# LayerXcom/zero-chain

Measured on NVIDIA H100. Metric: g1_msm_mops_2^20, higher is better.
Workload: dtype u32-limb Montgomery (Fq 12x32, Fr 8x32), integer

## Files before the change

zero_chain_b200/csrc/engine.cu:

```cuda
#define ZK_SEMI_HOT 1
#include "internal.h"
#include "msm_driver.cuh"

using namespace zkmsm;

static thread_local char g_err[512] = "";
void zk_set_error(const char *fmt, ...) {
    va_list ap; va_start(ap, fmt); vsnprintf(g_err, sizeof(g_err), fmt, ap); va_end(ap);
    (void)cudaGetLastError();
}
extern "C" const char *zk_last_error(void) { return g_err; }
extern "C" const char *zk_version(void) { return "zkb200 0.1 (sm_90a)"; }
extern "C" int zk_device_count(void) {
    int n = 0;
    if (cudaGetDeviceCount(&n) != cudaSuccess) { cudaGetLastError(); return 0; }
    return n;
}
int zk_use_device(zk_ctx *ctx) { ZK_CUDA(cudaSetDevice(ctx->device)); return ZK_OK; }

extern "C" int zk_ctx_create(int device, void *stream, zk_ctx **out) {
    if (!out) { zk_set_error("zk_ctx_create: out is NULL"); return ZK_ERR_INVALID; }
    int n = zk_device_count();
    if (n == 0) { zk_set_error("no CUDA device: libzkb200 has no CPU fallback"); return ZK_ERR_CUDA; }
    if (device < 0 || device >= n) { zk_set_error("device %d out of range (%d devices)", device, n); return ZK_ERR_INVALID; }
    ZK_CUDA(cudaSetDevice(device));
    zk_ctx *c = new zk_ctx();
    c->device = device;
    if (stream) { c->stream = (cudaStream_t)stream; c->own_stream = false; }
    else { ZK_CUDA(cudaStreamCreateWithFlags(&c->stream, cudaStreamNonBlocking)); c->own_stream = true; }
    cudaDeviceProp prop;
    ZK_CUDA(cudaGetDeviceProperties(&prop, device));
    c->sm_count = prop.multiProcessorCount;
    ZK_CUDA(cudaMalloc(&c->d_err, 32 * sizeof(int)));
    ZK_CUDA(cudaMemsetAsync(c->d_err, 0, 32 * sizeof(int), c->stream));
    c->h_pinned_cap = 1 << 20;
    ZK_CUDA(cudaMallocHost(&c->h_pinned, c->h_pinned_cap));
    *out = c;
    return ZK_OK;
}
extern "C" void zk_ctx_destroy(zk_ctx *c) {
    if (!c) return;
    if (c->aux) { zk_ctx_destroy(c->aux); c->aux = nullptr; }
    if (c->aux2) { zk_ctx_destroy(c->aux2); c->aux2 = nullptr; }
    if (c->aux3) { zk_ctx_destroy(c->aux3); c->aux3 = nullptr; }
    cudaSetDevice(c->device);
    cudaStreamSynchronize(c->stream);
    DevBuf *bufs[] = {&c->scalars, &c->digits, &c->tile_hist, &c->tile_off, &c->sizes, &c->bucket_off, &c->task_off, &c->scan_scratch,
                      &c->sorted, &c->partials, &c->buckets, &c->red_part, &c->red_x, &c->result, &c->out_bytes, &c->stage_a, &c->stage_b,
                      &c->stage_c, &c->ntt_tmp, &c->g_a, &c->g_b, &c->g_c, &c->g_h, &c->g_scal, &c->g_misc,
                      &c->aff_pts0, &c->aff_pts1, &c->aff_scratch, &c->aff_off0, &c->aff_off1, &c->aff_sizes0, &c->aff_sizes1, &c->aff_srcs, &c->aff_tot, &c->red_rows, &c->g_scal2, &c->g_scal3, &c->sorted2, &c->coarse_off, &c->coarse_sizes, &c->task_order, &c->len_hist, &c->heavy_list, &c->red_tmp,
                      &c->v_pts, &c->v_stat, &c->v_coef, &c->v_f, &c->v_part, &c->v_io, &c->v_jj,
                      &c->eg_table, &c->eg_index, &c->jm, &c->bal, &c->bal_io};
    for (DevBuf *b : bufs) b->release();
    for (NttSlot &sl : c->ntt_slots) { sl.w.release(); sl.g.release(); sl.gi.release(); sl.consts.release(); }
    if (c->tail) { cudaStreamSynchronize(c->tail); cudaStreamDestroy(c->tail); cudaEventDestroy(c->ev_front); cudaEventDestroy(c->ev_tail); }
    if (c->d_err) cudaFree(c->d_err);
    if (c->h_pinned) cudaFreeHost(c->h_pinned);
    if (c->own_stream) cudaStreamDestroy(c->stream);
    delete c;
}
extern "C" int zk_ctx_set_opt(zk_ctx *c, int opt, long value) {
    if (!c) { zk_set_error("zk_ctx_set_opt: NULL ctx"); return ZK_ERR_INVALID; }
    for (zk_ctx *x : {c, c->aux, c->aux2, c->aux3}) {
        if (!x) continue;
        if (opt == ZK_OPT_AFFINE_MIN_ENTRIES) x->opts.ba_min_entries = value;
        else if (opt == ZK_OPT_AFFINE_LEVELS) x->opts.ba_levels = value;
        else if (opt == ZK_OPT_VERIFY_LANES) x->opts.verify_lanes = value;
        else { zk_set_error("zk_ctx_set_opt: unknown option %d", opt); return ZK_ERR_INVALID; }
    }
    return ZK_OK;
}
extern "C" int zk_ctx_sync(zk_ctx *c) { ZK_TRY(zk_use_device(c)); return zk_check_err_flag(c); }
extern "C" void *zk_ctx_stream(zk_ctx *c) { return (void *)c->stream; }

int zk_check_err_flag(zk_ctx *ctx) {
    int e[3] = {0, 0, 0};
    ZK_CUDA(cudaMemcpyAsync(e, ctx->d_err, sizeof(e), cudaMemcpyDeviceToHost, ctx->stream));
    ZK_CUDA(cudaStreamSynchronize(ctx->stream));
    if (e[0] || e[1] || e[ZK_ERR_SLOT_ACCOUNT]) {
        ZK_CUDA(cudaMemsetAsync(ctx->d_err, 0, sizeof(e), ctx->stream));
        if (e[0]) { zk_set_error("scalar not canonical (>= r)"); return ZK_ERR_NOT_CANONICAL; }
        if (e[ZK_ERR_SLOT_ACCOUNT]) {
            zk_set_error("account %u: a stored ciphertext fails Ciphertext::read", ~(uint32_t)e[ZK_ERR_SLOT_ACCOUNT]);
// ... 333 lines not shown
```

zero_chain_b200/csrc/internal.h:

```cpp
#pragma once
#include <cuda_runtime.h>
#include <stdarg.h>
#include <stdint.h>
#include <stdio.h>
#include <string.h>
#include <string>
#include <vector>
#include "../../include/zkb200.h"

void zk_set_error(const char *fmt, ...);
#define ZK_CUDA(call)                                                                                  \
    do {                                                                                               \
        cudaError_t e__ = (call);                                                                      \
        if (e__ != cudaSuccess) {                                                                      \
            zk_set_error("%s:%d: %s -> %s", __FILE__, __LINE__, #call, cudaGetErrorString(e__));       \
            return ZK_ERR_CUDA;                                                                        \
        }                                                                                              \
    } while (0)
#define ZK_TRY(call) do { int r__ = (call); if (r__ != ZK_OK) return r__; } while (0)

struct DevBuf {
    void *p = nullptr;
    size_t cap = 0;
    int reserve(size_t bytes) {
// ... 5 lines not shown
        if (e != cudaSuccess) { zk_set_error("cudaMalloc(%zu) failed: %s", want, cudaGetErrorString(e)); return ZK_ERR_CUDA; }
        cap = want;
        return ZK_OK;
    }
    void release() { if (p) cudaFree(p); p = nullptr; cap = 0; }
    template <class T> T *as() const { return reinterpret_cast<T *>(p); }
};

struct Carve {
    uint8_t *base = nullptr;
    size_t off = 0;
    template <class T> T *take(size_t count) {
        T *p = reinterpret_cast<T *>(base ? base + off : nullptr);
        off += (count * sizeof(T) + 255) & ~(size_t)255;
        return p;
    }
};

struct NttSlot { unsigned log_n = 0; bool valid = false; uint64_t last_use = 0; DevBuf w, g, gi, consts; };

struct zk_opts {
    long ba_min_entries = 1l << 22;
    long ba_levels = -1;
    long verify_lanes = 1;
};

struct zk_ctx {
    zk_opts opts;
    int device = 0;
    cudaStream_t stream = nullptr;
    bool own_stream = false;
    int sm_count = 0;
    int *d_err = nullptr;
    DevBuf aff_pts0, aff_pts1, aff_scratch, aff_off0, aff_off1, aff_sizes0, aff_sizes1, aff_srcs, aff_tot;
    DevBuf scalars, digits, tile_hist, tile_off, sizes, bucket_off, task_off, scan_scratch, sorted, partials, buckets, red_part, red_x, red_rows, sorted2, coarse_off, coarse_sizes, task_order, len_hist, heavy_list, red_tmp, result, out_bytes;
    bool len_hist_zeroed = false;
    DevBuf stage_a, stage_b, stage_c;
    DevBuf ntt_tmp;
    NttSlot ntt_slots[4];
    uint64_t ntt_clock = 0;
    bool ntt_attr_done = false;
    DevBuf g_a, g_b, g_c, g_h, g_scal, g_misc;
    DevBuf v_pts, v_stat, v_coef, v_f, v_part, v_io;
    DevBuf v_jj;
    DevBuf eg_table, eg_index;
    bool eg_ready = false;
    DevBuf bal, bal_io;
    DevBuf jm;
    bool prof_on = false;
    std::vector<cudaEvent_t> prof_events;
    zk_ctx *aux2 = nullptr;
    zk_ctx *aux3 = nullptr;
    DevBuf g_scal3;
    zk_ctx *aux = nullptr;
    DevBuf g_scal2;
    cudaStream_t tail = nullptr;
    cudaEvent_t ev_front = nullptr, ev_tail = nullptr;
    bool split_tail = false;
    size_t pending_bytes = 0;
    uint8_t *h_pinned = nullptr;
    size_t h_pinned_cap = 0;
};

struct zk_bases {
    int group = 1;
    int device = 0;
    size_t n = 0;
// ... 38 lines not shown
```

zero_chain_b200/csrc/msm_accum.cuh:

```cuda
#pragma once
#include <cuda_runtime.h>
#include <stdint.h>
#include "curve.cuh"

namespace zkmsm {

constexpr int TASK_LEN_MAX = 64;
constexpr int TASK_LEN_MIN = 16;

template <class F>
__device__ __forceinline__ Affine<F> load_affine(const Affine<F> *__restrict__ p) {
    Affine<F> r;
    const uint4 *s = reinterpret_cast<const uint4 *>(p);
    uint4 *d = reinterpret_cast<uint4 *>(&r);
#pragma unroll
    for (int k = 0; k < (int)(sizeof(Affine<F>) / 16); k++) d[k] = __ldg(s + k);
    return r;
}
template <class F, int MINB>
__global__ void __launch_bounds__(128, MINB) k_accumulate(const Affine<F> *__restrict__ bases, const uint32_t *__restrict__ sorted,
                                                    const uint32_t *__restrict__ bucket_off, const uint32_t *__restrict__ task_off,
                                                    uint32_t n_buckets, const uint32_t *__restrict__ order, XYZZ<F> *__restrict__ partials) {
    uint32_t t = blockIdx.x * blockDim.x + threadIdx.x;
    uint32_t n_tasks = task_off[n_buckets];
    if (t >= n_tasks) return;
    if (order) t = order[t];
    uint32_t lo = 0, hi = n_buckets;
    while (hi - lo > 1) { uint32_t mid = (lo + hi) >> 1; if (task_off[mid] <= t) lo = mid; else hi = mid; }
    uint32_t b = lo, s = t - task_off[b];
    uint32_t nt = task_off[b + 1] - task_off[b], b0 = bucket_off[b], size = bucket_off[b + 1] - b0;
    uint32_t len = (size + nt - 1) / nt;
    uint32_t e0 = b0 + s * len, e1 = e0 + len;
    if (e1 > b0 + size) e1 = b0 + size;
    if (e0 >= e1) { partials[t] = XYZZ<F>::inf(); return; }
    XYZZ<F> acc = XYZZ<F>::inf();
    constexpr int VEC = (int)(sizeof(Affine<F>) / 16);
    __shared__ uint4 stage[128 * VEC];
    uint4 *slot = stage + threadIdx.x * VEC;
    const uint32_t slot_addr = (uint32_t)__cvta_generic_to_shared(slot);
    auto prefetch = [&](uint32_t c) {
        const uint4 *src = reinterpret_cast<const uint4 *>(bases + (c & 0x7fffffffu));
#pragma unroll
        for (int k = 0; k < VEC; k++)
            asm volatile("cp.async.cg.shared.global [%0], [%1], 16;" ::"r"(slot_addr + 16u * k), "l"(src + k) : "memory");
        asm volatile("cp.async.commit_group;" ::: "memory");
    };
    uint32_t code = sorted ? sorted[e0] : e0;
    prefetch(code);
    for (uint32_t e = e0; e < e1; e++) {
        asm volatile("cp.async.wait_group 0;" ::: "memory");
        Affine<F> p;
        {
            uint4 *d = reinterpret_cast<uint4 *>(&p);
#pragma unroll
            for (int k = 0; k < VEC; k++) d[k] = slot[k];
        }
        bool neg = code >> 31;
        if (e + 1 < e1) { code = sorted ? sorted[e + 1] : e + 1; prefetch(code); }
        p.y = p.y.cneg(neg);
        acc.add_mixed(p);
    }
    partials[t] = acc;
}
}
```

zero_chain_b200/csrc/msm_batchaff.cuh:

```cuda
#pragma once
#include <cuda_runtime.h>
#include <stdint.h>
#include "curve.cuh"
#include "msm_affine_core.cuh"
#include "msm_warp_scan.cuh"

namespace zkmsm {

constexpr int BA_T = 128;
constexpr int BA_K = 32;
constexpr int BA_MINB = 4;
constexpr int BA_MAX_LEVELS = 8;
constexpr int BA_INV_T = 512;
constexpr uint32_t BA_NONE = 0xffffffffu;

static __global__ void k_half_sizes(const uint32_t *__restrict__ off_in, uint32_t *__restrict__ sizes_out, uint32_t n_buckets) {
    uint32_t b = blockIdx.x * blockDim.x + threadIdx.x;
    if (b < n_buckets) sizes_out[b] = (off_in[b + 1] - off_in[b] + 1) >> 1;
}

template <class F>
__device__ __forceinline__ void ba_store_f(F *dst, const F &v) {
    const uint4 *s = reinterpret_cast<const uint4 *>(&v);
    uint4 *d = reinterpret_cast<uint4 *>(dst);
#pragma unroll
    for (int k = 0; k < (int)(sizeof(F) / 16); k++) d[k] = s[k];
}
template <class F>
__device__ __forceinline__ F ba_load_f(const F *src) {
    F v;
    const uint4 *s = reinterpret_cast<const uint4 *>(src);
    uint4 *d = reinterpret_cast<uint4 *>(&v);
#pragma unroll
    for (int k = 0; k < (int)(sizeof(F) / 16); k++) d[k] = s[k];
    return v;
}
template <class F, bool FIRST>
__device__ __forceinline__ const Affine<F> *ba_addr(const Affine<F> *pts, uint32_t code) { return pts + (FIRST ? (code & 0x7fffffffu) : code); }
template <class F, bool FIRST>
__device__ __forceinline__ Affine<F> ba_load_point(const Affine<F> *pts, uint32_t code) {
    Affine<F> p;
    const uint4 *s = reinterpret_cast<const uint4 *>(ba_addr<F, FIRST>(pts, code));
    uint4 *d = reinterpret_cast<uint4 *>(&p);
#pragma unroll
    for (int k = 0; k < (int)(sizeof(Affine<F>) / 16); k++) d[k] = __ldg(s + k);
    if (FIRST) p.y = p.y.cneg(code >> 31);
    return p;
}

template <class F, bool FIRST>
__device__ __forceinline__ F ba_load_x(const Affine<F> *pts, uint32_t code) {
    F x;
    const uint4 *s = reinterpret_cast<const uint4 *>(ba_addr<F, FIRST>(pts, code));
    uint4 *d = reinterpret_cast<uint4 *>(&x);
#pragma unroll
    for (int k = 0; k < (int)(sizeof(F) / 16); k++) d[k] = __ldg(s + k);
    return x;
}
template <class F, bool FIRST>
__global__ void __launch_bounds__(BA_T, 4) k_ba_forward(const Affine<F> *__restrict__ in_pts, const uint32_t *__restrict__ sorted,
                                                         const uint32_t *__restrict__ off_in, const uint32_t *__restrict__ off_out, uint32_t n_buckets, int K,
                                                         F *__restrict__ prefix, uint2 *__restrict__ srcs, F *__restrict__ block_totals) {
    const uint32_t total = off_out[n_buckets];
    const uint32_t n_blocks = (total + BA_T * K - 1) / (BA_T * K);
    if (blockIdx.x >= n_blocks) return;
    const int t = threadIdx.x;
    const size_t T_total = (size_t)gridDim.x * BA_T, tid = (size_t)blockIdx.x * BA_T + t;
    const uint32_t o0 = (uint32_t)tid * K;
    F run = F::one();
    if (o0 < total) {
        const uint32_t o1 = o0 + K < total ? o0 + K : total;
        {
            uint32_t lo = 0, hi = n_buckets;
            while (hi - lo > 1) { uint32_t mid = (lo + hi) >> 1; if (off_out[mid] <= o0) lo = mid; else hi = mid; }
            uint32_t b = lo, b_end = off_out[b + 1], b_out0 = off_out[b], b_in0 = off_in[b], b_sz = off_in[b + 1] - b_in0;
            for (uint32_t o = o0; o < o1; o++) {
                while (o >= b_end) { b++; b_out0 = b_end; b_end = off_out[b + 1]; b_in0 = off_in[b]; b_sz = off_in[b + 1] - b_in0; }
                const uint32_t j = o - b_out0, i0 = b_in0 + 2 * j;
                const bool has1 = 2 * j + 1 < b_sz;
                uint2 src;
                src.x = FIRST ? sorted[i0] : i0;
                src.y = has1 ? (FIRST ? sorted[i0 + 1] : i0 + 1) : BA_NONE;
                srcs[o] = src;
            }
        }
        uint2 s0 = srcs[o0], s1 = o0 + 1 < o1 ? srcs[o0 + 1] : make_uint2(0, BA_NONE);
        F xa0 = ba_load_x<F, FIRST>(in_pts, s0.x), xa1 = s0.y != BA_NONE ? ba_load_x<F, FIRST>(in_pts, s0.y) : F::zero();
        F xb0 = F::zero(), xb1 = F::zero();
        if (o0 + 1 < o1) { xb0 = ba_load_x<F, FIRST>(in_pts, s1.x); if (s1.y != BA_NONE) xb1 = ba_load_x<F, FIRST>(in_pts, s1.y); }
        for (uint32_t o = o0; o < o1; o++) {
            const uint2 cur = s0;
            const F x0 = xa0, x1 = xa1;
            s0 = s1; xa0 = xb0; xa1 = xb1;
            if (o + 2 < o1) {
                s1 = srcs[o + 2];
                xb0 = ba_load_x<F, FIRST>(in_pts, s1.x);
                if (s1.y != BA_NONE) xb1 = ba_load_x<F, FIRST>(in_pts, s1.y);
            }
            ba_store_f(prefix + (size_t)(o - o0) * T_total + tid, run);
            if (cur.y == BA_NONE) continue;
            F den = x1 - x0;
            if (den.is_zero() || x0.is_zero() || x1.is_zero()) {
                Affine<F> p0 = ba_load_point<F, FIRST>(in_pts, cur.x), p1 = ba_load_point<F, FIRST>(in_pts, cur.y);
                if (pair_classify(p0, p1, true, den) > PAIR_DBL) continue;
            }
            run = run * den;
        }
    }
    F others, all;
    ba_warp_products(run, others, all);
    ba_store_f(prefix + (size_t)K * T_total + tid, others);
    if ((t & 31) == 0) ba_store_f(block_totals + (tid >> 5), all);
}

template <class F>
__global__ void __launch_bounds__(BA_INV_T) k_ba_invert(const F *__restrict__ totals, const uint32_t *__restrict__ off_out, uint32_t n_buckets, int K,
                                                        F *__restrict__ scratch, F *__restrict__ inv_out) {
    extern __shared__ unsigned char ba_smem[];
    F *node = reinterpret_cast<F *>(ba_smem);
    const uint32_t total = off_out[n_buckets];
    const uint32_t n = ((total + BA_T * K - 1) / (BA_T * K)) * (BA_T / 32);
    const int t = threadIdx.x;
    const uint32_t per = (n + BA_INV_T - 1) / BA_INV_T, c0 = t * per, c1 = c0 + per < n ? c0 + per : n;
    F run = F::one();
    for (uint32_t i = c0; i < c1; i++) { ba_store_f(scratch + i, run); run = run * ba_load_f(totals + i); }
    node[BA_INV_T + t] = run;
    for (int s = BA_INV_T / 2; s >= 1; s >>= 1) {
        __syncthreads();
        if (t < s) node[s + t] = node[2 * (s + t)] * node[2 * (s + t) + 1];
    }
    __syncthreads();
    if (t == 0) node[1] = node[1].inverse();
    for (int s = 1; s < BA_INV_T; s <<= 1) {
        __syncthreads();
        if (t < s) {
            F inv = node[s + t], l = node[2 * (s + t)], r = node[2 * (s + t) + 1];
            node[2 * (s + t)] = inv * r;
            node[2 * (s + t) + 1] = inv * l;
        }
    }
    __syncthreads();
    F inv = node[BA_INV_T + t];
    for (uint32_t i = c1; i-- > c0;) {
        F v = ba_load_f(totals + i);
        ba_store_f(inv_out + i, inv * ba_load_f(scratch + i));
        inv = inv * v;
    }
}

template <class F, bool FIRST, int MINB>
__global__ void __launch_bounds__(BA_T, MINB) k_ba_backward(const Affine<F> *__restrict__ in_pts, const uint32_t *__restrict__ off_out, uint32_t n_buckets, int K,
                                                             const F *__restrict__ prefix, const uint2 *__restrict__ srcs, const F *__restrict__ block_inv,
                                                             Affine<F> *__restrict__ out_pts) {
    constexpr int PV = (int)(sizeof(Affine<F>) / 16), FV = (int)(sizeof(F) / 16);
    extern __shared__ unsigned char ba_smem[];
    uint4 *stage = reinterpret_cast<uint4 *>(ba_smem);
    const uint32_t total = off_out[n_buckets];
    const uint32_t n_blocks = (total + BA_T * K - 1) / (BA_T * K);
    if (blockIdx.x >= n_blocks) return;
    const int t = threadIdx.x;
    const size_t T_total = (size_t)gridDim.x * BA_T, tid = (size_t)blockIdx.x * BA_T + t;
    const uint32_t o0 = (uint32_t)tid * K;
    if (o0 >= total) return;
    F inv = ba_load_f(block_inv + (tid >> 5)) * ba_load_f(prefix + (size_t)K * T_total + tid);
    const uint32_t o1 = o0 + K < total ? o0 + K : total;
    uint4 *slot = stage + t;
    auto prefetch = [&](uint32_t o) {
        uint2 src = srcs[o];
        const uint4 *a = reinterpret_cast<const uint4 *>(ba_addr<F, FIRST>(in_pts, src.x));
        const uint4 *b = reinterpret_cast<const uint4 *>(ba_addr<F, FIRST>(in_pts, src.y == BA_NONE ? src.x : src.y));
        const uint4 *c = reinterpret_cast<const uint4 *>(prefix + (size_t)(o - o0) * T_total + tid);
#pragma unroll
        for (int v = 0; v < PV; v++) {
            asm volatile("cp.async.cg.shared.global [%0], [%1], 16;" ::"r"((uint32_t)__cvta_generic_to_shared(slot + v * BA_T)), "l"(a + v) : "memory");
            asm volatile("cp.async.cg.shared.global [%0], [%1], 16;" ::"r"((uint32_t)__cvta_generic_to_shared(slot + (PV + v) * BA_T)), "l"(b + v) : "memory");
        }
#pragma unroll
        for (int v = 0; v < FV; v++)
            asm volatile("cp.async.cg.shared.global [%0], [%1], 16;" ::"r"((uint32_t)__cvta_generic_to_shared(slot + (2 * PV + v) * BA_T)), "l"(c + v) : "memory");
        asm volatile("cp.async.commit_group;" ::: "memory");
        return src;
    };
    uint2 src = prefetch(o1 - 1);
    for (uint32_t o = o1; o-- > o0;) {
        asm volatile("cp.async.wait_group 0;" ::: "memory");
        Affine<F> p0, p1;
        F pre;
        {
            uint4 *d0 = reinterpret_cast<uint4 *>(&p0), *d1 = reinterpret_cast<uint4 *>(&p1), *d2 = reinterpret_cast<uint4 *>(&pre);
#pragma unroll
            for (int v = 0; v < PV; v++) { d0[v] = slot[v * BA_T]; d1[v] = slot[(PV + v) * BA_T]; }
#pragma unroll
            for (int v = 0; v < FV; v++) d2[v] = slot[(2 * PV + v) * BA_T];
        }
        const uint2 cur = src;
        if (o > o0) src = prefetch(o - 1);
        const bool has1 = cur.y != BA_NONE;
        if (FIRST) { p0.y = p0.y.cneg(cur.x >> 31); if (has1) p1.y = p1.y.cneg(cur.y >> 31); }
        if (!has1) p1 = Affine<F>::inf();
        F den;
        const int mode = pair_classify(p0, p1, has1, den);
        F dinv = F::one();
        if (mode <= PAIR_DBL) { dinv = inv * pre; inv = inv * den; }
        Affine<F> r = pair_finish(mode, p0, p1, dinv);
        uint4 *dst = reinterpret_cast<uint4 *>(out_pts + o);
        const uint4 *rs = reinterpret_cast<const uint4 *>(&r);
#pragma unroll
        for (int v = 0; v < PV; v++) dst[v] = rs[v];
    }
}

template <class F> constexpr size_t ba_smem_forward() { return 0; }
template <class F> constexpr size_t ba_smem_backward() { return (size_t)BA_T * (2 * sizeof(Affine<F>) + sizeof(F)); }
template <class F> constexpr size_t ba_smem_invert() { return 2 * BA_INV_T * sizeof(F); }

}
```

zero_chain_b200/csrc/msm_driver.cuh:

```cuda
#pragma once
#include "internal.h"
#include "msm.cuh"
#include "msm_batchaff.cuh"
#include "codec.cuh"
#include <stdlib.h>

namespace zkmsm {

template <class F>
int build_tables_t(zk_ctx *ctx, zk_bases *b) {
    unsigned thr = 128, blk = (unsigned)((b->n + thr * PRE_K - 1) / (thr * PRE_K));
    k_precompute<F><<<blk, thr, 0, ctx->stream>>>((Affine<F> *)b->d_tbl, (uint32_t)b->n, b->c, b->W);
    ZK_CUDA(cudaGetLastError());
    return ZK_OK;
}

template <class F>
int msm_run_t(zk_ctx *ctx, const zk_bases *b, const uint32_t *d_scalars, size_t n, size_t batch) {
    cudaStream_t st = ctx->stream;
    const int c = b->c, W = b->W, nbins = 1 << (c - 1);
    const bool tables = b->tables;
    if (!tables && batch != 1) { zk_set_error("batched MSM needs precomputed tables"); return ZK_ERR_INVALID; }
    const size_t n_dom = tables ? batch : (size_t)W;
    const uint64_t e_dom = tables ? (uint64_t)n * W : (uint64_t)n;
// ... 29 lines not shown
    ZK_TRY(ctx->red_x.reserve(2 * n_dom * n_bits * pt));
    ZK_TRY(ctx->result.reserve((n_dom + batch + 1) * pt));

    uint32_t *digits = ctx->digits.as<uint32_t>();
    {
        dim3 g((unsigned)((n + 255) / 256), (unsigned)batch);
        k_msm_digits<<<g, 256, 0, st>>>(d_scalars, (uint32_t)n, c, W, digits, ctx->d_err);
    }
    const size_t SB = n_dom * (size_t)sort_bins;
    if (smem > 48 * 1024) {
        ZK_CUDA(cudaFuncSetAttribute(k_tile_hist, cudaFuncAttributeMaxDynamicSharedMemorySize, (int)smem));
        ZK_CUDA(cudaFuncSetAttribute(k_scatter, cudaFuncAttributeMaxDynamicSharedMemorySize, (int)smem));
    }
    dim3 gs((unsigned)tiles, (unsigned)n_dom);
    if (!two_level) {
        k_tile_hist<<<gs, SORT_THREADS, smem, st>>>(digits, e_dom, nbins, 0, ctx->tile_hist.as<uint32_t>(), tiles, tile_len, false);
        k_col_scan<<<(unsigned)((NB + 255) / 256), 256, 0, st>>>(ctx->tile_hist.as<uint32_t>(), ctx->tile_off.as<uint32_t>(), ctx->sizes.as<uint32_t>(),
                                                                nbins, tiles, (int)n_dom);
        exclusive_scan<false>(ctx->sizes.as<uint32_t>(), ctx->bucket_off.as<uint32_t>(), NB, ctx->scan_scratch.as<uint32_t>(), st);
        k_scatter<<<gs, SORT_THREADS, smem, st>>>(digits, e_dom, nbins, ctx->tile_off.as<uint32_t>(), ctx->bucket_off.as<uint32_t>(),
                                                  ctx->sorted.as<uint32_t>(), tiles, tile_len);
    } else {
        ZK_TRY(ctx->sorted2.reserve(E * sizeof(uint2)));
        ZK_TRY(ctx->coarse_off.reserve((SB + 1) * 4)); ZK_TRY(ctx->coarse_sizes.reserve((SB + 1) * 4));
        k_tile_hist<<<gs, COARSE_THREADS, smem, st>>>(digits, e_dom, sort_bins, low, ctx->tile_hist.as<uint32_t>(), tiles, tile_len, true);
        k_bin_scan<<<(unsigned)SB, COARSE_THREADS, 0, st>>>(ctx->tile_hist.as<uint32_t>(), ctx->tile_off.as<uint32_t>(), ctx->coarse_sizes.as<uint32_t>(), tiles);
        exclusive_scan<false>(ctx->coarse_sizes.as<uint32_t>(), ctx->coarse_off.as<uint32_t>(), SB, ctx->scan_scratch.as<uint32_t>(), st);
        k_coarse_scatter<<<gs, COARSE_THREADS, 0, st>>>(digits, e_dom, low, ctx->tile_off.as<uint32_t>(), ctx->coarse_off.as<uint32_t>(),
                                                        ctx->sorted2.as<uint2>(), tiles, tile_len);
        ZK_CUDA(cudaFuncSetAttribute(k_fine_sort, cudaFuncAttributeMaxDynamicSharedMemorySize, FINE_STAGE * 4));
        k_fine_sort<<<dim3(512, (unsigned)n_dom), 1024, FINE_STAGE * 4, st>>>(ctx->sorted2.as<uint2>(), ctx->coarse_off.as<uint32_t>(), 512, low,
                                                                 ctx->sizes.as<uint32_t>(), ctx->bucket_off.as<uint32_t>(), ctx->sorted.as<uint32_t>());
    }
    const Affine<F> *cur_pts = (const Affine<F> *)b->d_tbl;
    const uint32_t *cur_sorted = ctx->sorted.as<uint32_t>(), *cur_off = ctx->bucket_off.as<uint32_t>(), *cur_sizes = ctx->sizes.as<uint32_t>();
    struct ProfPair {
        cudaEvent_t a = nullptr, b = nullptr; bool kept = false;
        ~ProfPair() { if (!kept) { if (a) cudaEventDestroy(a); if (b) cudaEventDestroy(b); } }
    } prof;
    cudaEvent_t &ev0 = prof.a, &ev1 = prof.b;
    {
        int levels = 0;
        if (ctx->opts.ba_min_entries >= 0 && (long)E >= ctx->opts.ba_min_entries) {
            if (ctx->opts.ba_levels >= 0) levels = (int)(ctx->opts.ba_levels < BA_MAX_LEVELS ? ctx->opts.ba_levels : BA_MAX_LEVELS);
            else for (size_t avg = E / NB; avg >= 12 && levels < BA_MAX_LEVELS; avg >>= 1) levels++;
        }
        if (ctx->prof_on && levels > 0) { cudaEventCreate(&ev0); cudaEventCreate(&ev1); cudaEventRecord(ev0, st); }
        size_t in_max = E;
        int minb = BA_MINB, k_force = 0;
        (void)minb;
#ifdef ZK_EXPERIMENTS
        if (const char *e = getenv("ZK_BA_MINB")) minb = atoi(e);
        if (const char *e = getenv("ZK_BA_K")) k_force = atoi(e);
#endif
        DevBuf *pts_buf[2] = {&ctx->aff_pts0, &ctx->aff_pts1}, *off_buf[2] = {&ctx->aff_off0, &ctx->aff_off1}, *sz_buf[2] = {&ctx->aff_sizes0, &ctx->aff_sizes1};
        if (levels > 0) {
            if (ba_smem_backward<F>() > 48 * 1024) {
                ZK_CUDA(cudaFuncSetAttribute(k_ba_backward<F, true, BA_MINB>, cudaFuncAttributeMaxDynamicSharedMemorySize, (int)ba_smem_backward<F>()));
                ZK_CUDA(cudaFuncSetAttribute(k_ba_backward<F, false, BA_MINB>, cudaFuncAttributeMaxDynamicSharedMemorySize, (int)ba_smem_backward<F>()));
#ifdef ZK_EXPERIMENTS
                ZK_CUDA(cudaFuncSetAttribute(k_ba_backward<F, true, 3>, cudaFuncAttributeMaxDynamicSharedMemorySize, (int)ba_smem_backward<F>()));
                ZK_CUDA(cudaFuncSetAttribute(k_ba_backward<F, false, 3>, cudaFuncAttributeMaxDynamicSharedMemorySize, (int)ba_smem_backward<F>()));
#endif
            }
            if (ba_smem_invert<F>() > 48 * 1024)
                ZK_CUDA(cudaFuncSetAttribute(k_ba_invert<F>, cudaFuncAttributeMaxDynamicSharedMemorySize, (int)ba_smem_invert<F>()));
        }
        for (int l = 0; l < levels; l++) {
            const size_t out_max = (in_max + NB) / 2 + 1;
            int K = BA_K;
            if (k_force > 0) K = k_force;
            const unsigned grid = (unsigned)((out_max + (size_t)BA_T * K - 1) / ((size_t)BA_T * K));
            const size_t T_total = (size_t)grid * BA_T;
            DevBuf *pts_o = pts_buf[l & 1], *off_o = off_buf[l & 1], *sz_o = sz_buf[l & 1];
            ZK_TRY(pts_o->reserve(out_max * sizeof(Affine<F>)));
            ZK_TRY(off_o->reserve((NB + 1) * 4)); ZK_TRY(sz_o->reserve((NB + 1) * 4));
            ZK_TRY(ctx->aff_scratch.reserve((size_t)(K + 1) * T_total * sizeof(F)));
            ZK_TRY(ctx->aff_srcs.reserve(out_max * sizeof(uint2)));
            const size_t n_tot = (size_t)grid * (BA_T / 32);
            ZK_TRY(ctx->aff_tot.reserve(3 * n_tot * sizeof(F)));
            F *tot = ctx->aff_tot.as<F>(), *tot_scr = tot + n_tot, *tot_inv = tot + 2 * n_tot;
            k_half_sizes<<<(unsigned)((NB + 255) / 256), 256, 0, st>>>(cur_off, sz_o->as<uint32_t>(), (uint32_t)NB);
            exclusive_scan<false>(sz_o->as<uint32_t>(), off_o->as<uint32_t>(), NB, ctx->scan_scratch.as<uint32_t>(), st);
            const uint32_t *off_out = off_o->as<uint32_t>();
            if (l == 0)
                k_ba_forward<F, true><<<grid, BA_T, ba_smem_forward<F>(), st>>>(cur_pts, cur_sorted, cur_off, off_out, (uint32_t)NB, K, ctx->aff_scratch.as<F>(),
                                                                               ctx->aff_srcs.as<uint2>(), tot);
            else
                k_ba_forward<F, false><<<grid, BA_T, ba_smem_forward<F>(), st>>>(cur_pts, nullptr, cur_off, off_out, (uint32_t)NB, K, ctx->aff_scratch.as<F>(),
                                                                                ctx->aff_srcs.as<uint2>(), tot);
            k_ba_invert<F><<<1, BA_INV_T, ba_smem_invert<F>(), st>>>(tot, off_out, (uint32_t)NB, K, tot_scr, tot_inv);
            const int Kb = K;
#define ZK_BA_BWD(FIRST_, MB_) k_ba_backward<F, FIRST_, MB_><<<grid, BA_T, ba_smem_backward<F>(), st>>>(cur_pts, off_out, (uint32_t)NB, Kb, ctx->aff_scratch.as<F>(), \
                                                                                                    ctx->aff_srcs.as<uint2>(), tot_inv, pts_o->as<Affine<F>>())
#ifdef ZK_EXPERIMENTS
            if (minb == 3) { if (l == 0) ZK_BA_BWD(true, 3); else ZK_BA_BWD(false, 3); } else
#endif
            { if (l == 0) ZK_BA_BWD(true, BA_MINB); else ZK_BA_BWD(false, BA_MINB); }
#undef ZK_BA_BWD
            cur_pts = pts_o->as<Affine<F>>(); cur_sorted = nullptr;
            cur_off = off_out; cur_sizes = sz_o->as<uint32_t>();
            in_max = out_max;
        }
    }
    uint32_t *d_task_len = (uint32_t *)(ctx->d_err + 8);
    const uint32_t capacity = (uint32_t)ctx->sm_count * 3u * 128u;
    unsigned long long *d_work = (unsigned long long *)(ctx->d_err + (sizeof(F) == sizeof(Fq) ? 10 : 12));
    k_pick_task_len<<<1, 1, 0, st>>>(cur_off + NB, ctx->bucket_off.as<uint32_t>() + NB, d_task_len, capacity, d_work, d_work + 2);
    exclusive_scan<true>(cur_sizes, ctx->task_off.as<uint32_t>(), NB, ctx->scan_scratch.as<uint32_t>(), st, d_task_len);
    XYZZ<F> *partials = ctx->partials.as<XYZZ<F>>(), *buckets = ctx->buckets.as<XYZZ<F>>();
    const uint32_t *order = nullptr;
    {
        bool want = E / NB < 256;
        if (want) {
            ZK_TRY(ctx->task_order.reserve(t_max * 4)); ZK_TRY(ctx->len_hist.reserve(2 * LEN_BINS * 4 + 64));
            uint32_t *gh = ctx->len_hist.as<uint32_t>(), *cur = gh + LEN_BINS;
            if (!ctx->len_hist_zeroed) { ZK_CUDA(cudaMemsetAsync(gh, 0, 2 * LEN_BINS * 4, st)); ctx->len_hist_zeroed = true; }
            unsigned nb = (unsigned)((NB + LEN_BLOCK - 1) / LEN_BLOCK);
            k_len_hist<<<nb, LEN_BLOCK, 0, st>>>(cur_off, ctx->task_off.as<uint32_t>(), (uint32_t)NB, gh);
            k_len_scan<<<1, LEN_BINS, 0, st>>>(gh, cur);
            k_len_place<<<nb, LEN_BLOCK, 0, st>>>(cur_off, ctx->task_off.as<uint32_t>(), (uint32_t)NB, cur, ctx->task_order.as<uint32_t>());
            order = ctx->task_order.as<uint32_t>();
        }
    }
    {
        const Affine<F> *tb = cur_pts;
        const uint32_t *so = cur_sorted, *bo = cur_off, *to = ctx->task_off.as<uint32_t>();
        unsigned grid = (unsigned)((t_max + 127) / 128);
        if (ctx->prof_on && !ev0) { cudaEventCreate(&ev0); cudaEventCreate(&ev1); cudaEventRecord(ev0, st); }
        k_accumulate<F, 3><<<grid, 128, 0, st>>>(tb, so, bo, to, (uint32_t)NB, order, partials);
    }
    if (ctx->prof_on) { cudaEventRecord(ev1, st); ctx->prof_events.push_back(ev0); ctx->prof_events.push_back(ev1); prof.kept = true; }
    if (ctx->split_tail) {
        ZK_CUDA(cudaEventRecord(ctx->ev_front, st));
        ZK_CUDA(cudaStreamWaitEvent(ctx->tail, ctx->ev_front, 0));
        st = ctx->tail;
    }
    const size_t sm_warp = 4 * 32 * pt;
    if (sm_warp > 48 * 1024) {
        ZK_CUDA(cudaFuncSetAttribute(k_combine_warp<F>, cudaFuncAttributeMaxDynamicSharedMemorySize, (int)sm_warp));
        ZK_CUDA(cudaFuncSetAttribute(k_bit_sums<F>, cudaFuncAttributeMaxDynamicSharedMemorySize, (int)sm_warp));
        ZK_CUDA(cudaFuncSetAttribute(k_sum_points<F>, cudaFuncAttributeMaxDynamicSharedMemorySize, (int)sm_warp));
        ZK_CUDA(cudaFuncSetAttribute(k_finish_bits<F>, cudaFuncAttributeMaxDynamicSharedMemorySize, (int)sm_warp));
    }
    ZK_TRY(ctx->heavy_list.reserve((NB + 1) * 4));
    uint32_t *heavy_count = d_task_len + 1;
    k_combine_serial<F><<<(unsigned)((NB + 127) / 128), 128, 0, st>>>(partials, ctx->task_off.as<uint32_t>(), (uint32_t)NB, buckets,
                                                                      ctx->heavy_list.as<uint32_t>(), heavy_count);
    k_combine_warp<F><<<(unsigned)(2 * ctx->sm_count), 128, sm_warp, st>>>(partials, ctx->task_off.as<uint32_t>(), ctx->heavy_list.as<uint32_t>(), heavy_count, buckets);
    XYZZ<F> *part = ctx->red_part.as<XYZZ<F>>(), *X = ctx->red_x.as<XYZZ<F>>(), *R = ctx->result.as<XYZZ<F>>();
    auto bit_reduce = [&](const XYZZ<F> *Bk, int N, int bits, size_t nd, XYZZ<F> *out) {
        int slices = (N / 2 + RED_SLICE / 2 - 1) / (RED_SLICE / 2); if (slices < 1) slices = 1;
        size_t n_w = (size_t)slices * bits * nd, n_g = nd * (size_t)bits;
        k_bit_sums<F><<<(unsigned)((n_w * 32 + RED_T - 1) / RED_T), RED_T, sm_warp, st>>>(Bk, N, slices, bits, (int)nd, part);
        k_sum_points<F><<<(unsigned)((n_g * 32 + RED_T - 1) / RED_T), RED_T, sm_warp, st>>>(part, slices, (int)n_g, X);
        k_finish_bits<F><<<(unsigned)nd, FIN_WARPS * 32, 2 * FIN_WARPS * sizeof(XYZZ<F>), st>>>(X, bits, (int)nd, out);
    };
    XYZZ<F> *Rdom = tables ? R : R + 1;
    if ((n_dom >= 8 && c >= 7) || (tables && c > 16)) {
        const int s = (c - 1) / 2, nr = nbins >> s, nc = (1 << s) - 1;
        ZK_TRY(ctx->red_rows.reserve(2 * n_dom * (size_t)nr * pt));
        ZK_TRY(ctx->result.reserve((3 * n_dom + batch + 4) * pt));
        R = ctx->result.as<XYZZ<F>>();
// ... 42 lines not shown
```

Measured before the change: 156.3.

## Split batch-affine points into SoA x/y arrays, interleave lanes, drop srcs buffer

Intermediate points produced by the batch-affine reduction levels are now stored as separate x and y arrays instead of interleaved affine structs. Each thread's work items are strided by 32 across a warp, so neighbouring lanes touch consecutive outputs. The srcs buffer is gone: forward and backward kernels now recompute source indices by walking bucket offsets. The aim is coalesced stores and loads and less global traffic, at the cost of a repeated binary search and offset walk in the backward kernel.

```diff
diff --git a/zero_chain_b200/csrc/engine.cu b/zero_chain_b200/csrc/engine.cu
--- a/zero_chain_b200/csrc/engine.cu
+++ b/zero_chain_b200/csrc/engine.cu
@@ -48,7 +48,7 @@
     DevBuf *bufs[] = {&c->scalars, &c->digits, &c->tile_hist, &c->tile_off, &c->sizes, &c->bucket_off, &c->task_off, &c->scan_scratch,
                       &c->sorted, &c->partials, &c->buckets, &c->red_part, &c->red_x, &c->result, &c->out_bytes, &c->stage_a, &c->stage_b,
                       &c->stage_c, &c->ntt_tmp, &c->g_a, &c->g_b, &c->g_c, &c->g_h, &c->g_scal, &c->g_misc,
-                      &c->aff_pts0, &c->aff_pts1, &c->aff_scratch, &c->aff_off0, &c->aff_off1, &c->aff_sizes0, &c->aff_sizes1, &c->aff_srcs, &c->aff_tot, &c->red_rows, &c->g_scal2, &c->g_scal3, &c->sorted2, &c->coarse_off, &c->coarse_sizes, &c->task_order, &c->len_hist, &c->heavy_list, &c->red_tmp,
+                      &c->aff_pts0, &c->aff_pts1, &c->aff_scratch, &c->aff_off0, &c->aff_off1, &c->aff_sizes0, &c->aff_sizes1, &c->aff_tot, &c->red_rows, &c->g_scal2, &c->g_scal3, &c->sorted2, &c->coarse_off, &c->coarse_sizes, &c->task_order, &c->len_hist, &c->heavy_list, &c->red_tmp,
                       &c->v_pts, &c->v_stat, &c->v_coef, &c->v_f, &c->v_part, &c->v_io, &c->v_jj,
                       &c->eg_table, &c->eg_index, &c->jm, &c->bal, &c->bal_io};
     for (DevBuf *b : bufs) b->release();
diff --git a/zero_chain_b200/csrc/internal.h b/zero_chain_b200/csrc/internal.h
--- a/zero_chain_b200/csrc/internal.h
+++ b/zero_chain_b200/csrc/internal.h
@@ -61,7 +61,7 @@
     bool own_stream = false;
     int sm_count = 0;
     int *d_err = nullptr;
-    DevBuf aff_pts0, aff_pts1, aff_scratch, aff_off0, aff_off1, aff_sizes0, aff_sizes1, aff_srcs, aff_tot;
+    DevBuf aff_pts0, aff_pts1, aff_scratch, aff_off0, aff_off1, aff_sizes0, aff_sizes1, aff_tot;
     DevBuf scalars, digits, tile_hist, tile_off, sizes, bucket_off, task_off, scan_scratch, sorted, partials, buckets, red_part, red_x, red_rows, sorted2, coarse_off, coarse_sizes, task_order, len_hist, heavy_list, red_tmp, result, out_bytes;
     bool len_hist_zeroed = false;
     DevBuf stage_a, stage_b, stage_c;
diff --git a/zero_chain_b200/csrc/msm_accum.cuh b/zero_chain_b200/csrc/msm_accum.cuh
--- a/zero_chain_b200/csrc/msm_accum.cuh
+++ b/zero_chain_b200/csrc/msm_accum.cuh
@@ -18,7 +18,7 @@
     return r;
 }
 template <class F, int MINB>
-__global__ void __launch_bounds__(128, MINB) k_accumulate(const Affine<F> *__restrict__ bases, const uint32_t *__restrict__ sorted,
+__global__ void __launch_bounds__(128, MINB) k_accumulate(const F *__restrict__ xs, const F *__restrict__ ys, const uint32_t *__restrict__ sorted,
                                                     const uint32_t *__restrict__ bucket_off, const uint32_t *__restrict__ task_off,
                                                     uint32_t n_buckets, const uint32_t *__restrict__ order, XYZZ<F> *__restrict__ partials) {
     uint32_t t = blockIdx.x * blockDim.x + threadIdx.x;
@@ -34,15 +34,18 @@
     if (e1 > b0 + size) e1 = b0 + size;
     if (e0 >= e1) { partials[t] = XYZZ<F>::inf(); return; }
     XYZZ<F> acc = XYZZ<F>::inf();
-    constexpr int VEC = (int)(sizeof(Affine<F>) / 16);
+    constexpr int VEC = (int)(sizeof(Affine<F>) / 16), FV = (int)(sizeof(F) / 16);
     __shared__ uint4 stage[128 * VEC];
     uint4 *slot = stage + threadIdx.x * VEC;
     const uint32_t slot_addr = (uint32_t)__cvta_generic_to_shared(slot);
     auto prefetch = [&](uint32_t c) {
-        const uint4 *src = reinterpret_cast<const uint4 *>(bases + (c & 0x7fffffffu));
+        const F *px = ys ? xs + c : xs + 2 * (size_t)(c & 0x7fffffffu), *py = ys ? ys + c : px + 1;
+        const uint4 *sx = reinterpret_cast<const uint4 *>(px), *sy = reinterpret_cast<const uint4 *>(py);
 #pragma unroll
-        for (int k = 0; k < VEC; k++)
-            asm volatile("cp.async.cg.shared.global [%0], [%1], 16;" ::"r"(slot_addr + 16u * k), "l"(src + k) : "memory");
+        for (int k = 0; k < FV; k++) {
+            asm volatile("cp.async.cg.shared.global [%0], [%1], 16;" ::"r"(slot_addr + 16u * k), "l"(sx + k) : "memory");
+            asm volatile("cp.async.cg.shared.global [%0], [%1], 16;" ::"r"(slot_addr + 16u * (FV + k)), "l"(sy + k) : "memory");
+        }
         asm volatile("cp.async.commit_group;" ::: "memory");
     };
     uint32_t code = sorted ? sorted[e0] : e0;
diff --git a/zero_chain_b200/csrc/msm_batchaff.cuh b/zero_chain_b200/csrc/msm_batchaff.cuh
--- a/zero_chain_b200/csrc/msm_batchaff.cuh
+++ b/zero_chain_b200/csrc/msm_batchaff.cuh
@@ -35,73 +35,96 @@
     for (int k = 0; k < (int)(sizeof(F) / 16); k++) d[k] = s[k];
     return v;
 }
-template <class F, bool FIRST>
-__device__ __forceinline__ const Affine<F> *ba_addr(const Affine<F> *pts, uint32_t code) { return pts + (FIRST ? (code & 0x7fffffffu) : code); }
-template <class F, bool FIRST>
-__device__ __forceinline__ Affine<F> ba_load_point(const Affine<F> *pts, uint32_t code) {
+template <class F>
+__device__ __forceinline__ F ba_ldg_f(const F *src) {
+    F v;
+    const uint4 *s = reinterpret_cast<const uint4 *>(src);
+    uint4 *d = reinterpret_cast<uint4 *>(&v);
+#pragma unroll
+    for (int k = 0; k < (int)(sizeof(F) / 16); k++) d[k] = __ldg(s + k);
+    return v;
+}
+template <class F, bool FIRST>
+__device__ __forceinline__ const F *ba_x(const F *in_x, uint32_t code) { return FIRST ? in_x + 2 * (size_t)(code & 0x7fffffffu) : in_x + code; }
+template <class F, bool FIRST>
+__device__ __forceinline__ const F *ba_y(const F *in_x, const F *in_y, uint32_t code) { return FIRST ? ba_x<F, FIRST>(in_x, code) + 1 : in_y + code; }
+template <class F, bool FIRST>
+__device__ __forceinline__ Affine<F> ba_load_point(const F *in_x, const F *in_y, uint32_t code) {
     Affine<F> p;
-    const uint4 *s = reinterpret_cast<const uint4 *>(ba_addr<F, FIRST>(pts, code));
-    uint4 *d = reinterpret_cast<uint4 *>(&p);
-#pragma unroll
-    for (int k = 0; k < (int)(sizeof(Affine<F>) / 16); k++) d[k] = __ldg(s + k);
+    p.x = ba_ldg_f(ba_x<F, FIRST>(in_x, code));
+    p.y = ba_ldg_f(ba_y<F, FIRST>(in_x, in_y, code));
     if (FIRST) p.y = p.y.cneg(code >> 31);
     return p;
 }
 
-template <class F, bool FIRST>
-__device__ __forceinline__ F ba_load_x(const Affine<F> *pts, uint32_t code) {
-    F x;
-    const uint4 *s = reinterpret_cast<const uint4 *>(ba_addr<F, FIRST>(pts, code));
-    uint4 *d = reinterpret_cast<uint4 *>(&x);
-#pragma unroll
-    for (int k = 0; k < (int)(sizeof(F) / 16); k++) d[k] = __ldg(s + k);
-    return x;
-}
-template <class F, bool FIRST>
-__global__ void __launch_bounds__(BA_T, 4) k_ba_forward(const Affine<F> *__restrict__ in_pts, const uint32_t *__restrict__ sorted,
+struct BaWalk {
+    uint32_t b, out0, out1, in0, in1;
+    __device__ __forceinline__ BaWalk(const uint32_t *off_in, const uint32_t *off_out, uint32_t n_buckets, uint32_t o) {
+        uint32_t lo = 0, hi = n_buckets;
+        while (hi - lo > 1) { uint32_t mid = (lo + hi) >> 1; if (off_out[mid] <= o) lo = mid; else hi = mid; }
+        b = lo; out0 = off_out[b]; out1 = off_out[b + 1]; in0 = off_in[b]; in1 = off_in[b + 1];
+    }
+    __device__ __forceinline__ void forward(const uint32_t *off_in, const uint32_t *off_out, uint32_t o) {
+        while (o >= out1) { b++; out0 = out1; out1 = off_out[b + 1]; in0 = in1; in1 = off_in[b + 1]; }
+    }
+    __device__ __forceinline__ void backward(const uint32_t *off_in, const uint32_t *off_out, uint32_t o) {
+        while (o < out0) { b--; out1 = out0; out0 = off_out[b]; in1 = in0; in0 = off_in[b]; }
+    }
+    template <bool FIRST>
+    __device__ __forceinline__ uint2 src(const uint32_t *sorted, uint32_t o) const {
+        const uint32_t i0 = in0 + 2 * (o - out0);
+        uint2 s;
+        s.x = FIRST ? sorted[i0] : i0;
+        s.y = i0 + 1 < in1 ? (FIRST ? sorted[i0 + 1] : i0 + 1) : BA_NONE;
+        return s;
+    }
+};
+__device__ __forceinline__ uint32_t ba_lane_first(size_t tid, int K) { return (uint32_t)(tid >> 5) * 32u * (uint32_t)K + (uint32_t)(tid & 31); }
+__device__ __forceinline__ int ba_lane_count(uint32_t total, uint32_t oa, int K) {
+    if (oa >= total) return 0;
+    const uint32_t n = (total - oa + 31) >> 5;
+    return n < (uint32_t)K ? (int)n : K;
+}
+
+template <class F, bool FIRST>
+__global__ void __launch_bounds__(BA_T, 4) k_ba_forward(const F *__restrict__ in_x, const F *__restrict__ in_y, const uint32_t *__restrict__ sorted,
                                                          const uint32_t *__restrict__ off_in, const uint32_t *__restrict__ off_out, uint32_t n_buckets, int K,
-                                                         F *__restrict__ prefix, uint2 *__restrict__ srcs, F *__restrict__ block_totals) {
+                                                         F *__restrict__ prefix, F *__restrict__ block_totals) {
     const uint32_t total = off_out[n_buckets];
     const uint32_t n_blocks = (total + BA_T * K - 1) / (BA_T * K);
     if (blockIdx.x >= n_blocks) return;
     const int t = threadIdx.x;
     const size_t T_total = (size_t)gridDim.x * BA_T, tid = (size_t)blockIdx.x * BA_T + t;
-    const uint32_t o0 = (uint32_t)tid * K;
+    const uint32_t oa = ba_lane_first(tid, K);
+    const int n = ba_lane_count(total, oa, K);
     F run = F::one();
-    if (o0 < total) {
-        const uint32_t o1 = o0 + K < total ? o0 + K : total;
-        {
-            uint32_t lo = 0, hi = n_buckets;
-            while (hi - lo > 1) { uint32_t mid = (lo + hi) >> 1; if (off_out[mid] <= o0) lo = mid; else hi = mid; }
-            uint32_t b = lo, b_end = off_out[b + 1], b_out0 = off_out[b], b_in0 = off_in[b], b_sz = off_in[b + 1] - b_in0;
-            for (uint32_t o = o0; o < o1; o++) {
-                while (o >= b_end) { b++; b_out0 = b_end; b_end = off_out[b + 1]; b_in0 = off_in[b]; b_sz = off_in[b + 1] - b_in0; }
-                const uint32_t j = o - b_out0, i0 = b_in0 + 2 * j;
-                const bool has1 = 2 * j + 1 < b_sz;
-                uint2 src;
-                src.x = FIRST ? sorted[i0] : i0;
-                src.y = has1 ? (FIRST ? sorted[i0 + 1] : i0 + 1) : BA_NONE;
-                srcs[o] = src;
-            }
-        }
-        uint2 s0 = srcs[o0], s1 = o0 + 1 < o1 ? srcs[o0 + 1] : make_uint2(0, BA_NONE);
-        F xa0 = ba_load_x<F, FIRST>(in_pts, s0.x), xa1 = s0.y != BA_NONE ? ba_load_x<F, FIRST>(in_pts, s0.y) : F::zero();
+    if (n > 0) {
+        BaWalk w(off_in, off_out, n_buckets, oa);
+        uint2 s0 = w.src<FIRST>(sorted, oa), s1 = make_uint2(0, BA_NONE);
+        F xa0 = ba_ldg_f(ba_x<F, FIRST>(in_x, s0.x)), xa1 = s0.y != BA_NONE ? ba_ldg_f(ba_x<F, FIRST>(in_x, s0.y)) : F::zero();
         F xb0 = F::zero(), xb1 = F::zero();
-        if (o0 + 1 < o1) { xb0 = ba_load_x<F, FIRST>(in_pts, s1.x); if (s1.y != BA_NONE) xb1 = ba_load_x<F, FIRST>(in_pts, s1.y); }
-        for (uint32_t o = o0; o < o1; o++) {
+        if (n > 1) {
+            w.forward(off_in, off_out, oa + 32);
+            s1 = w.src<FIRST>(sorted, oa + 32);
+            xb0 = ba_ldg_f(ba_x<F, FIRST>(in_x, s1.x));
+            if (s1.y != BA_NONE) xb1 = ba_ldg_f(ba_x<F, FIRST>(in_x, s1.y));
+        }
+        for (int k = 0; k < n; k++) {
             const uint2 cur = s0;
             const F x0 = xa0, x1 = xa1;
             s0 = s1; xa0 = xb0; xa1 = xb1;
-            if (o + 2 < o1) {
-                s1 = srcs[o + 2];
-                xb0 = ba_load_x<F, FIRST>(in_pts, s1.x);
-                if (s1.y != BA_NONE) xb1 = ba_load_x<F, FIRST>(in_pts, s1.y);
+            if (k + 2 < n) {
+                const uint32_t o = oa + 32u * (uint32_t)(k + 2);
+                w.forward(off_in, off_out, o);
+                s1 = w.src<FIRST>(sorted, o);
+                xb0 = ba_ldg_f(ba_x<F, FIRST>(in_x, s1.x));
+                if (s1.y != BA_NONE) xb1 = ba_ldg_f(ba_x<F, FIRST>(in_x, s1.y));
             }
-            ba_store_f(prefix + (size_t)(o - o0) * T_total + tid, run);
+            ba_store_f(prefix + (size_t)k * T_total + tid, run);
             if (cur.y == BA_NONE) continue;
             F den = x1 - x0;
             if (den.is_zero() || x0.is_zero() || x1.is_zero()) {
-                Affine<F> p0 = ba_load_point<F, FIRST>(in_pts, cur.x), p1 = ba_load_point<F, FIRST>(in_pts, cur.y);
+                Affine<F> p0 = ba_load_point<F, FIRST>(in_x, in_y, cur.x), p1 = ba_load_point<F, FIRST>(in_x, in_y, cur.y);
                 if (pair_classify(p0, p1, true, den) > PAIR_DBL) continue;
             }
             run = run * den;
@@ -149,9 +172,10 @@
 }
 
 template <class F, bool FIRST, int MINB>
-__global__ void __launch_bounds__(BA_T, MINB) k_ba_backward(const Affine<F> *__restrict__ in_pts, const uint32_t *__restrict__ off_out, uint32_t n_buckets, int K,
-                                                             const F *__restrict__ prefix, const uint2 *__restrict__ srcs, const F *__restrict__ block_inv,
-                                                             Affine<F> *__restrict__ out_pts) {
+__global__ void __launch_bounds__(BA_T, MINB) k_ba_backward(const F *__restrict__ in_x, const F *__restrict__ in_y, const uint32_t *__restrict__ sorted,
+                                                             const uint32_t *__restrict__ off_in, const uint32_t *__restrict__ off_out, uint32_t n_buckets, int K,
+                                                             const F *__restrict__ prefix, const F *__restrict__ block_inv,
+                                                             F *__restrict__ out_x, F *__restrict__ out_y) {
     constexpr int PV = (int)(sizeof(Affine<F>) / 16), FV = (int)(sizeof(F) / 16);
     extern __shared__ unsigned char ba_smem[];
     uint4 *stage = reinterpret_cast<uint4 *>(ba_smem);
@@ -160,29 +184,30 @@
     if (blockIdx.x >= n_blocks) return;
     const int t = threadIdx.x;
     const size_t T_total = (size_t)gridDim.x * BA_T, tid = (size_t)blockIdx.x * BA_T + t;
-    const uint32_t o0 = (uint32_t)tid * K;
-    if (o0 >= total) return;
+    const uint32_t oa = ba_lane_first(tid, K);
+    const int n = ba_lane_count(total, oa, K);
+    if (n == 0) return;
     F inv = ba_load_f(block_inv + (tid >> 5)) * ba_load_f(prefix + (size_t)K * T_total + tid);
-    const uint32_t o1 = o0 + K < total ? o0 + K : total;
     uint4 *slot = stage + t;
-    auto prefetch = [&](uint32_t o) {
-        uint2 src = srcs[o];
-        const uint4 *a = reinterpret_cast<const uint4 *>(ba_addr<F, FIRST>(in_pts, src.x));
-        const uint4 *b = reinterpret_cast<const uint4 *>(ba_addr<F, FIRST>(in_pts, src.y == BA_NONE ? src.x : src.y));
-        const uint4 *c = reinterpret_cast<const uint4 *>(prefix + (size_t)(o - o0) * T_total + tid);
-#pragma unroll
-        for (int v = 0; v < PV; v++) {
-            asm volatile("cp.async.cg.shared.global [%0], [%1], 16;" ::"r"((uint32_t)__cvta_generic_to_shared(slot + v * BA_T)), "l"(a + v) : "memory");
-            asm volatile("cp.async.cg.shared.global [%0], [%1], 16;" ::"r"((uint32_t)__cvta_generic_to_shared(slot + (PV + v) * BA_T)), "l"(b + v) : "memory");
-        }
-#pragma unroll
-        for (int v = 0; v < FV; v++)
-            asm volatile("cp.async.cg.shared.global [%0], [%1], 16;" ::"r"((uint32_t)__cvta_generic_to_shared(slot + (2 * PV + v) * BA_T)), "l"(c + v) : "memory");
+    auto copy = [&](int v, const F *src) {
+        const uint4 *s = reinterpret_cast<const uint4 *>(src);
+#pragma unroll
+        for (int u = 0; u < FV; u++)
+            asm volatile("cp.async.cg.shared.global [%0], [%1], 16;" ::"r"((uint32_t)__cvta_generic_to_shared(slot + (v + u) * BA_T)), "l"(s + u) : "memory");
+    };
+    auto prefetch = [&](int k, uint2 src) {
+        const uint32_t c1 = src.y == BA_NONE ? src.x : src.y;
+        copy(0, ba_x<F, FIRST>(in_x, src.x));
+        copy(FV, ba_y<F, FIRST>(in_x, in_y, src.x));
+        copy(PV, ba_x<F, FIRST>(in_x, c1));
+        copy(PV + FV, ba_y<F, FIRST>(in_x, in_y, c1));
+        copy(2 * PV, prefix + (size_t)k * T_total + tid);
         asm volatile("cp.async.commit_group;" ::: "memory");
-        return src;
     };
-    uint2 src = prefetch(o1 - 1);
-    for (uint32_t o = o1; o-- > o0;) {
+    BaWalk w(off_in, off_out, n_buckets, oa + 32u * (uint32_t)(n - 1));
+    uint2 src = w.src<FIRST>(sorted, oa + 32u * (uint32_t)(n - 1));
+    prefetch(n - 1, src);
+    for (int k = n; k-- > 0;) {
         asm volatile("cp.async.wait_group 0;" ::: "memory");
         Affine<F> p0, p1;
         F pre;
@@ -194,7 +219,12 @@
             for (int v = 0; v < FV; v++) d2[v] = slot[(2 * PV + v) * BA_T];
         }
         const uint2 cur = src;
-        if (o > o0) src = prefetch(o - 1);
+        if (k > 0) {
+            const uint32_t o = oa + 32u * (uint32_t)(k - 1);
+            w.backward(off_in, off_out, o);
+            src = w.src<FIRST>(sorted, o);
+            prefetch(k - 1, src);
+        }
         const bool has1 = cur.y != BA_NONE;
         if (FIRST) { p0.y = p0.y.cneg(cur.x >> 31); if (has1) p1.y = p1.y.cneg(cur.y >> 31); }
         if (!has1) p1 = Affine<F>::inf();
@@ -203,10 +233,9 @@
         F dinv = F::one();
         if (mode <= PAIR_DBL) { dinv = inv * pre; inv = inv * den; }
         Affine<F> r = pair_finish(mode, p0, p1, dinv);
-        uint4 *dst = reinterpret_cast<uint4 *>(out_pts + o);
-        const uint4 *rs = reinterpret_cast<const uint4 *>(&r);
-#pragma unroll
-        for (int v = 0; v < PV; v++) dst[v] = rs[v];
+        const uint32_t o = oa + 32u * (uint32_t)k;
+        ba_store_f(out_x + o, r.x);
+        ba_store_f(out_y + o, r.y);
     }
 }
 
diff --git a/zero_chain_b200/csrc/msm_driver.cuh b/zero_chain_b200/csrc/msm_driver.cuh
--- a/zero_chain_b200/csrc/msm_driver.cuh
+++ b/zero_chain_b200/csrc/msm_driver.cuh
@@ -85,7 +85,7 @@
         k_fine_sort<<<dim3(512, (unsigned)n_dom), 1024, FINE_STAGE * 4, st>>>(ctx->sorted2.as<uint2>(), ctx->coarse_off.as<uint32_t>(), 512, low,
                                                                  ctx->sizes.as<uint32_t>(), ctx->bucket_off.as<uint32_t>(), ctx->sorted.as<uint32_t>());
     }
-    const Affine<F> *cur_pts = (const Affine<F> *)b->d_tbl;
+    const F *cur_x = (const F *)b->d_tbl, *cur_y = nullptr;
     const uint32_t *cur_sorted = ctx->sorted.as<uint32_t>(), *cur_off = ctx->bucket_off.as<uint32_t>(), *cur_sizes = ctx->sizes.as<uint32_t>();
     struct ProfPair {
         cudaEvent_t a = nullptr, b = nullptr; bool kept = false;
@@ -127,9 +127,9 @@
             const size_t T_total = (size_t)grid * BA_T;
             DevBuf *pts_o = pts_buf[l & 1], *off_o = off_buf[l & 1], *sz_o = sz_buf[l & 1];
             ZK_TRY(pts_o->reserve(out_max * sizeof(Affine<F>)));
+            F *out_x = pts_o->as<F>(), *out_y = out_x + out_max;
             ZK_TRY(off_o->reserve((NB + 1) * 4)); ZK_TRY(sz_o->reserve((NB + 1) * 4));
             ZK_TRY(ctx->aff_scratch.reserve((size_t)(K + 1) * T_total * sizeof(F)));
-            ZK_TRY(ctx->aff_srcs.reserve(out_max * sizeof(uint2)));
             const size_t n_tot = (size_t)grid * (BA_T / 32);
             ZK_TRY(ctx->aff_tot.reserve(3 * n_tot * sizeof(F)));
             F *tot = ctx->aff_tot.as<F>(), *tot_scr = tot + n_tot, *tot_inv = tot + 2 * n_tot;
@@ -137,21 +137,19 @@
             exclusive_scan<false>(sz_o->as<uint32_t>(), off_o->as<uint32_t>(), NB, ctx->scan_scratch.as<uint32_t>(), st);
             const uint32_t *off_out = off_o->as<uint32_t>();
             if (l == 0)
-                k_ba_forward<F, true><<<grid, BA_T, ba_smem_forward<F>(), st>>>(cur_pts, cur_sorted, cur_off, off_out, (uint32_t)NB, K, ctx->aff_scratch.as<F>(),
-                                                                               ctx->aff_srcs.as<uint2>(), tot);
+                k_ba_forward<F, true><<<grid, BA_T, ba_smem_forward<F>(), st>>>(cur_x, cur_y, cur_sorted, cur_off, off_out, (uint32_t)NB, K, ctx->aff_scratch.as<F>(), tot);
             else
-                k_ba_forward<F, false><<<grid, BA_T, ba_smem_forward<F>(), st>>>(cur_pts, nullptr, cur_off, off_out, (uint32_t)NB, K, ctx->aff_scratch.as<F>(),
-                                                                                ctx->aff_srcs.as<uint2>(), tot);
+                k_ba_forward<F, false><<<grid, BA_T, ba_smem_forward<F>(), st>>>(cur_x, cur_y, nullptr, cur_off, off_out, (uint32_t)NB, K, ctx->aff_scratch.as<F>(), tot);
             k_ba_invert<F><<<1, BA_INV_T, ba_smem_invert<F>(), st>>>(tot, off_out, (uint32_t)NB, K, tot_scr, tot_inv);
             const int Kb = K;
-#define ZK_BA_BWD(FIRST_, MB_) k_ba_backward<F, FIRST_, MB_><<<grid, BA_T, ba_smem_backward<F>(), st>>>(cur_pts, off_out, (uint32_t)NB, Kb, ctx->aff_scratch.as<F>(), \
-                                                                                                    ctx->aff_srcs.as<uint2>(), tot_inv, pts_o->as<Affine<F>>())
+#define ZK_BA_BWD(FIRST_, MB_) k_ba_backward<F, FIRST_, MB_><<<grid, BA_T, ba_smem_backward<F>(), st>>>(cur_x, cur_y, cur_sorted, cur_off, off_out, (uint32_t)NB, Kb, \
+                                                                                                    ctx->aff_scratch.as<F>(), tot_inv, out_x, out_y)
 #ifdef ZK_EXPERIMENTS
             if (minb == 3) { if (l == 0) ZK_BA_BWD(true, 3); else ZK_BA_BWD(false, 3); } else
 #endif
             { if (l == 0) ZK_BA_BWD(true, BA_MINB); else ZK_BA_BWD(false, BA_MINB); }
 #undef ZK_BA_BWD
-            cur_pts = pts_o->as<Affine<F>>(); cur_sorted = nullptr;
+            cur_x = out_x; cur_y = out_y; cur_sorted = nullptr;
             cur_off = off_out; cur_sizes = sz_o->as<uint32_t>();
             in_max = out_max;
         }
@@ -177,11 +175,10 @@
         }
     }
     {
-        const Affine<F> *tb = cur_pts;
         const uint32_t *so = cur_sorted, *bo = cur_off, *to = ctx->task_off.as<uint32_t>();
         unsigned grid = (unsigned)((t_max + 127) / 128);
         if (ctx->prof_on && !ev0) { cudaEventCreate(&ev0); cudaEventCreate(&ev1); cudaEventRecord(ev0, st); }
-        k_accumulate<F, 3><<<grid, 128, 0, st>>>(tb, so, bo, to, (uint32_t)NB, order, partials);
+        k_accumulate<F, 3><<<grid, 128, 0, st>>>(cur_x, cur_y, so, bo, to, (uint32_t)NB, order, partials);
     }
     if (ctx->prof_on) { cudaEventRecord(ev1, st); ctx->prof_events.push_back(ev0); ctx->prof_events.push_back(ev1); prof.kept = true; }
     if (ctx->split_tail) {
```

Result: faster. 165.1, median of 6 (+5.6%).
